# ahuang73/HemoCell

Hardware: AMD Instinct MI355X
Metric: MLUPS + cell-vertex updates/s, 256^3 pipeflow 10% Hct (higher is better)
Workload: dtype f64

## Files before the change

### hemocell_amd/csrc/common.h

```cpp
#pragma once
#include <hip/hip_runtime.h>
#include <stdint.h>
#include <string>
#include <vector>
#include "../../include/hemocell_amd.h"

namespace hc {

void set_error(const std::string &msg);
int hip_fail(hipError_t e, const char *what, const char *file, int line);
hipStream_t stream();
hipStream_t comm_stream();
int fork();
void route(int side);
int join();
bool forked();

#define HC_HIP(call)                                                         \
  do {                                                                       \
    hipError_t e__ = (call);                                                 \
    if (e__ != hipSuccess) return hc::hip_fail(e__, #call, __FILE__, __LINE__); \
  } while (0)

#define HC_REQUIRE(cond, msg)                 \
  do {                                        \
    if (!(cond)) {                            \
      hc::set_error(std::string(msg));        \
      return HC_ERR_ARG;                      \
    }                                         \
  } while (0)

enum ProfKernel { PK_COLLIDE = 0, PK_SPREAD, PK_INTERP, PK_ADVANCE, PK_MECH, PK_COLLIDE_BESIDE, PK_LEES_EDWARDS, PK_COUNT };
struct ProfScope {
  int k; bool on;
  hipEvent_t a, b;
  explicit ProfScope(int kernel);
  ~ProfScope();
};

#define HC_CX {0, -1, 0, 0, -1, -1, -1, -1, 0, 0, 1, 0, 0, 1, 1, 1, 1, 0, 0}
#define HC_CY {0, 0, -1, 0, -1, 1, 0, 0, -1, -1, 0, 1, 0, 1, -1, 0, 0, 1, 1}
#define HC_CZ {0, 0, 0, -1, 0, 0, -1, 1, -1, 1, 0, 0, 1, 0, 0, 1, -1, 1, -1}

constexpr int HALO = 2;

constexpr int STAT_BLOCKS = 512;
struct StatAcc { double mn, mx, sum; long n; };
__device__ __forceinline__ void stat_add(StatAcc &a, double v) { a.mn = v < a.mn ? v : a.mn; a.mx = v > a.mx ? v : a.mx; a.sum += v; a.n++; }
__device__ __forceinline__ void stat_block_store(StatAcc a, double *partial ) {
  __shared__ double s_red[4][4];
#pragma unroll
  for (int off = 32; off > 0; off >>= 1) {
    const double mn = __shfl_xor(a.mn, off), mx = __shfl_xor(a.mx, off), sm = __shfl_xor(a.sum, off);
    const long n = __shfl_xor(a.n, off);
    a.mn = mn < a.mn ? mn : a.mn; a.mx = mx > a.mx ? mx : a.mx; a.sum += sm; a.n += n;
  }
  const int w = threadIdx.x >> 6;
  if ((threadIdx.x & 63) == 0) { s_red[w][0] = a.mn; s_red[w][1] = a.mx; s_red[w][2] = a.sum; s_red[w][3] = (double)a.n; }
  __syncthreads();
  if (threadIdx.x == 0) {
    double mn = s_red[0][0], mx = s_red[0][1], sm = s_red[0][2], n = s_red[0][3];
    for (int k = 1; k < (int)(blockDim.x >> 6); k++) { mn = s_red[k][0] < mn ? s_red[k][0] : mn; mx = s_red[k][1] > mx ? s_red[k][1] : mx; sm += s_red[k][2]; n += s_red[k][3]; }
    double *o = partial + 4 * blockIdx.x;
    o[0] = mn; o[1] = mx; o[2] = sm; o[3] = n;
  }
}
int stat_finish(const double *d_partial, double out[3], long *n, double *h_pinned = nullptr);

}

namespace hc {
struct BodyRegions { int n; int box[HC_MAX_FORCE_REGIONS][6]; double f[HC_MAX_FORCE_REGIONS][3]; };
#ifdef __HIPCC__
__device__ __forceinline__ void region_force(const BodyRegions &r, int xg, int y, int z, double &bx, double &by, double &bz) {
  for (int k = 0; k < r.n; k++) {
    const int *b = r.box[k];
    if (xg >= b[0] && xg <= b[1] && y >= b[2] && y <= b[3] && z >= b[4] && z <= b[5]) { bx = r.f[k][0]; by = r.f[k][1]; bz = r.f[k][2]; }
  }
}

__device__ __forceinline__ void zou_he_x(double f[HC_Q], int code, const double *__restrict__ val) {
  const int kind = code & 3;
  const long slot = code >> 2;
  const double s0 = f[0] + f[2] + f[3] + f[8] + f[9] + f[11] + f[12] + f[17] + f[18];
  const double sm = f[1] + f[4] + f[5] + f[6] + f[7];
  const double sp = f[10] + f[13] + f[14] + f[15] + f[16];
  const bool neg = (kind & 1) == 0;
  const double s_out = neg ? sm : sp;
  const double known = s0 + 2.0 * s_out + 1.0;
  double rho, ux, uy, uz;
  if (kind < 2) {
    ux = val[4 * slot]; uy = val[4 * slot + 1]; uz = val[4 * slot + 2];
    rho = neg ? known / (1.0 - ux) : known / (1.0 + ux);
  } else {
    rho = val[4 * slot + 3];
    ux = neg ? 1.0 - known / rho : known / rho - 1.0;
    uy = 0.0; uz = 0.0;
  }
  const double ny = 0.5 * ((f[11] + f[17] + f[18]) - (f[2] + f[8] + f[9])) - rho * uy / 3.0;
  const double nz = 0.5 * ((f[12] + f[9] + f[17]) - (f[3] + f[8] + f[18])) - rho * uz / 3.0;
  if (neg) {
    f[10] = f[1] + rho * ux / 3.0;
    f[13] = f[4] + rho * (ux + uy) / 6.0 - ny;
    f[14] = f[5] + rho * (ux - uy) / 6.0 + ny;
    f[15] = f[6] + rho * (ux + uz) / 6.0 - nz;
    f[16] = f[7] + rho * (ux - uz) / 6.0 + nz;
  } else {
    f[1] = f[10] - rho * ux / 3.0;
    f[4] = f[13] - rho * (ux + uy) / 6.0 + ny;
    f[5] = f[14] - rho * (ux - uy) / 6.0 - ny;
    f[6] = f[15] - rho * (ux + uz) / 6.0 + nz;
    f[7] = f[16] - rho * (ux - uz) / 6.0 - nz;
  }
}
#endif
}

struct hc_lattice {
  int nx, ny, nz;
  int periodic[3];
  int x0, nx_global, n_slabs;
  double omega;
  size_t plane;
  size_t xs;
  size_t npad;
  size_t qstride;
  double *f[2];
  int cur;
  double *force[3];
  int fcur;
  int ibm;
  uint8_t *fdirty[3];
  uint8_t fepoch[3];
  uint8_t *wallbrick; int nbx, nby, nbz;
  uint8_t *mask;
  std::vector<uint8_t> hmask;
  double body[3];
  hc::BodyRegions regions;
  double wall_u[4][3];
  int *row_z0, *row_cum, *blk_row;
  int nblk, max_active;
  double *scratch;
  size_t scratch_doubles;
  double *halo_u[2] = {nullptr, nullptr};
  bool halo_u_valid = false;
  bool le_on = false;
  double le_D = 0.0, le_d = 0.0, le_v_top = 0.0, le_v_bottom = 0.0;
  double *le_buf = nullptr;
  int *ob_code = nullptr;
  std::vector<int> ob_hcode;
  double *ob_val = nullptr;
  int ob_n = 0, ob_cap = 0;
  int *ob_list = nullptr; int ob_list_cap = 0;
  double *ob_out = nullptr; int ob_out_cap = 0;
};

namespace hc {
int lees_edwards_step(hc_lattice *L);
}

namespace hcs {
int iterate_slab(hc_lattice *L, hc_cells *C, long *iter, int n, int particle_timescale, int force_limit);
int collide_stream_slab(hc_lattice *L, int nsteps);
void lattice_destroyed(hc_lattice *L);
void halos_stale(hc_lattice *L);
void set_overlap(int on);
}
```

### hemocell_amd/csrc/lattice.hip

```cpp
#include "common.h"
#include "comm.h"
#include <algorithm>
#include <type_traits>

using namespace hc;

namespace {

struct LatArgs {
  const double *fin;
  double *fout;
  const double *Fin;
  double *Fzero;
  const uint8_t *mask;
  int nx, ny, nz;
  int plane;
  long xs;
  long npad;
  long qs;
  int x_begin;
  int x_split, x_jump;
  int wrap_x, per_y, per_z;
  double omega;
  double bx, by, bz;
  const int *row_z0, *row_cum, *blk_row;
  int nblk;
  int ibm;
  const uint8_t *dirty_in, *dirty_zero; uint8_t epoch_in, epoch_zero;
  double wall_u[4][3];
  int x0, nx_global;
  BodyRegions reg;
};

struct OpenArgs : LatArgs {
  const int *ob_code;
  const double *ob_val;
};
template <bool OPEN> using Args = std::conditional_t<OPEN, OpenArgs, LatArgs>;

__device__ __forceinline__ void body_at(const LatArgs &a, int x, int y, int z, double &bx, double &by, double &bz) {
  bx = a.bx; by = a.by; bz = a.bz;
  if (a.reg.n) region_force(a.reg, a.x0 + x, y, z, bx, by, bz);
}

struct Nbr {
  long xm, xp;
  int ym, yp, zm, zp;
  bool ym_ok, yp_ok, zm_ok, zp_ok;
};

__device__ __forceinline__ Nbr neighbours(const LatArgs &a, int x, int y, int z) {
  Nbr n;
  n.xm = -a.xs; n.xp = a.xs;
  if (a.wrap_x) {
    if (x == 0) n.xm = (long)(a.nx - 1) * a.xs;
    if (x == a.nx - 1) n.xp = -(long)(a.nx - 1) * a.xs;
  }
  n.ym = -a.nz; n.yp = a.nz; n.ym_ok = n.yp_ok = true;
  if (y == 0) { if (a.per_y) n.ym = (a.ny - 1) * a.nz; else n.ym_ok = false; }
  if (y == a.ny - 1) { if (a.per_y) n.yp = -(a.ny - 1) * a.nz; else n.yp_ok = false; }
  n.zm = -1; n.zp = 1; n.zm_ok = n.zp_ok = true;
  if (z == 0) { if (a.per_z) n.zm = a.nz - 1; else n.zm_ok = false; }
  if (z == a.nz - 1) { if (a.per_z) n.zp = -(a.nz - 1); else n.zp_ok = false; }
  return n;
}

template <int CX, int CY, int CZ>
__device__ __forceinline__ long src_off(const Nbr &n, bool &ok) {
  long off = 0; ok = true;
  if (CX == 1) off += n.xm; else if (CX == -1) off += n.xp;
  if (CY == 1) { off += n.ym; ok = ok && n.ym_ok; } else if (CY == -1) { off += n.yp; ok = ok && n.yp_ok; }
  if (CZ == 1) { off += n.zm; ok = ok && n.zm_ok; } else if (CZ == -1) { off += n.zp; ok = ok && n.zp_ok; }
  return off;
}
template <int CX, int CY, int CZ>
__device__ __forceinline__ long dst_off(const Nbr &n, bool &ok) {
  long off = 0; ok = true;
  if (CX == 1) off += n.xp; else if (CX == -1) off += n.xm;
  if (CY == 1) { off += n.yp; ok = ok && n.yp_ok; } else if (CY == -1) { off += n.ym; ok = ok && n.ym_ok; }
  if (CZ == 1) { off += n.zp; ok = ok && n.zp_ok; } else if (CZ == -1) { off += n.zm; ok = ok && n.zm_ok; }
  return off;
}

#define FOR_Q(M)                                                                                     \
  M(0, 0, 0, 0) M(1, -1, 0, 0) M(2, 0, -1, 0) M(3, 0, 0, -1) M(4, -1, -1, 0) M(5, -1, 1, 0)          \
  M(6, -1, 0, -1) M(7, -1, 0, 1) M(8, 0, -1, -1) M(9, 0, -1, 1) M(10, 1, 0, 0) M(11, 0, 1, 0)        \
  M(12, 0, 0, 1) M(13, 1, 1, 0) M(14, 1, -1, 0) M(15, 1, 0, 1) M(16, 1, 0, -1) M(17, 0, 1, 1)        \
  M(18, 0, 1, -1)

__device__ __forceinline__ constexpr double tq(int q) { return q == 0 ? 1. / 3. : ((q >= 1 && q <= 3) || (q >= 10 && q <= 12)) ? 1. / 18. : 1. / 36.; }

__device__ __forceinline__ void pull(const double *__restrict__ fin, long npad, long node, const Nbr &n, double f[HC_Q]) {
#define M(Q, CX, CY, CZ)                                   \
  {                                                        \
    bool ok; long off = src_off<CX, CY, CZ>(n, ok);        \
    f[Q] = ok ? fin[(long)Q * npad + node + off] : 0.0;    \
  }
  FOR_Q(M)
#undef M
}

template <bool OPEN>
__device__ __forceinline__ void complete_open(const Args<OPEN> &a, long node, double f[HC_Q]) {
  if constexpr (OPEN) {
    if (a.mask[node] == 0) {
      const int code = a.ob_code[node];
      if (code >= 0) zou_he_x(f, code, a.ob_val);
    }
  }
}

__device__ __forceinline__ void moments(const double f[HC_Q], double &rhoBar, double &jx, double &jy, double &jz) {
  double r = 0.0, x = 0.0, y = 0.0, z = 0.0;
#define M(Q, CX, CY, CZ)              \
  r += f[Q];                          \
  if (CX == 1) x += f[Q]; else if (CX == -1) x += -f[Q]; \
  if (CY == 1) y += f[Q]; else if (CY == -1) y += -f[Q]; \
  if (CZ == 1) z += f[Q]; else if (CZ == -1) z += -f[Q];
  FOR_Q(M)
#undef M
  rhoBar = r; jx = x; jy = y; jz = z;
}

template <int CX, int CY, int CZ>
__device__ __forceinline__ double cdot(double a0, double a1, double a2) {
  double s = 0.0; bool first = true;
  if (CX != 0) { s = (CX == 1 ? a0 : -a0); first = false; }
  if (CY != 0) { double t = (CY == 1 ? a1 : -a1); s = first ? t : s + t; first = false; }
  if (CZ != 0) { double t = (CZ == 1 ? a2 : -a2); s = first ? t : s + t; first = false; }
  return s;
}

__device__ __forceinline__ void collide_guo(double f[HC_Q], double Fx, double Fy, double Fz, double omega) {
  double rhoBar, j0, j1, j2;
  moments(f, rhoBar, j0, j1, j2);
  const double invRho = 1.0 / (1.0 + rhoBar);
  const double rho = 1.0 + rhoBar;
  const double u0 = j0 * invRho + Fx / 2.0, u1 = j1 * invRho + Fy / 2.0, u2 = j2 * invRho + Fz / 2.0;
  j0 = rho * u0; j1 = rho * u1; j2 = rho * u2;
  const double jSqr = j0 * j0 + j1 * j1 + j2 * j2;
  const double one_m_omega = 1.0 - omega;
  const double guo = 1.0 - omega / 2.0;
#define M(Q, CX, CY, CZ)                                                                     \
  {                                                                                          \
    const double c_j = cdot<CX, CY, CZ>(j0, j1, j2);                                         \
    const double feq = tq(Q) * (rhoBar + 3.0 * c_j + invRho * (4.5 * c_j * c_j - 1.5 * jSqr)); \
    f[Q] *= one_m_omega;                                                                     \
    f[Q] += omega * feq;                                                                     \
  }
  FOR_Q(M)
#undef M
#define M(Q, CX, CY, CZ)                                                                     \
  {                                                                                          \
    double c_u = cdot<CX, CY, CZ>(u0, u1, u2);                                               \
    c_u *= 9.0;                                                                              \
    double ft = (((double)CX - u0) * 3.0 + c_u * (double)CX) * Fx;                           \
    ft += (((double)CY - u1) * 3.0 + c_u * (double)CY) * Fy;                                 \
    ft += (((double)CZ - u2) * 3.0 + c_u * (double)CZ) * Fz;                                 \
    ft *= tq(Q);                                                                             \
    ft *= guo;                                                                               \
    f[Q] += ft;                                                                              \
  }
  FOR_Q(M)
#undef M
}

template <bool REGIONS, bool OPEN = false>
__global__ __launch_bounds__(256) void collide_stream_kernel(Args<OPEN> a) {
  const int x = a.x_begin + (int)blockIdx.y + ((int)blockIdx.y >= a.x_split ? a.x_jump : 0);
  const int xp = x + HALO;
  const int t = blockIdx.x * 256 + threadIdx.x;
  const int *cum = a.row_cum + (long)xp * (a.ny + 1);
  if (t >= cum[a.ny]) return;
  int lo = a.blk_row[(long)xp * (a.nblk + 1) + blockIdx.x], hi = a.blk_row[(long)xp * (a.nblk + 1) + blockIdx.x + 1];
  while (lo < hi) { const int mid = (lo + hi + 1) >> 1; if (cum[mid] <= t) lo = mid; else hi = mid - 1; }
  const int y = lo, z = a.row_z0[(long)xp * a.ny + y] + (t - cum[y]);
  const int p = y * a.nz + z;
  const long node = (long)(x + HALO) * a.xs + p;
  const uint8_t m = a.mask[node];
  if (m == 2) return;
  const Nbr n = neighbours(a, x, y, z);
  const bool fdirty = a.ibm && m == 0 && a.dirty_in[node >> 4] == a.epoch_in;
  double F0 = 0.0, F1 = 0.0, F2 = 0.0;
  if (fdirty) { F0 = a.Fin[3 * node]; F1 = a.Fin[3 * node + 1]; F2 = a.Fin[3 * node + 2]; }
  double f[HC_Q];
  pull(a.fin, a.qs, node, n, f);
  const bool wall = m != 0;
  if (wall) {
#pragma unroll
    for (int i = 1; i <= 9; i++) { double t = f[i]; f[i] = f[i + 9]; f[i + 9] = t; }
    if (m >= 3) {
      const double w0 = a.wall_u[m - 3][0], w1 = a.wall_u[m - 3][1], w2 = a.wall_u[m - 3][2];
#define M(Q, CX, CY, CZ)                                                                  \
      if (Q != 0) {                                                                       \
        constexpr int O = Q <= 9 ? Q + 9 : Q - 9;                                         \
        const double c_u = (double)CX * w0 + (double)CY * w1 + (double)CZ * w2;           \
        f[O] = f[O] - 6.0 * tq(Q) * c_u;                                                  \
      }
      FOR_Q(M)
#undef M
    }
  } else {
    double bx = a.bx, by = a.by, bz = a.bz;
    if (REGIONS) region_force(a.reg, a.x0 + x, y, z, bx, by, bz);
    double Fx = bx, Fy = by, Fz = bz;
    if (fdirty) {
      Fx = bx + F0; Fy = by + F1; Fz = bz + F2;
    }
    if constexpr (OPEN) {
      const int code = a.ob_code[node];
      if (code >= 0) zou_he_x(f, code, a.ob_val);
    }
    collide_guo(f, Fx, Fy, Fz, a.omega);
  }
#pragma unroll
  for (int q = 0; q < HC_Q; q++) __builtin_nontemporal_store(f[q], &a.fout[(long)q * a.qs + node]);
  if (a.ibm && a.dirty_zero[node >> 4] == a.epoch_zero) { a.Fzero[3 * node] = 0.0; a.Fzero[3 * node + 1] = 0.0; a.Fzero[3 * node + 2] = 0.0; }
}

__global__ void init_eq_kernel(LatArgs a, double rhoBar, double j0, double j1, double j2) {
  const int p = blockIdx.x * 256 + threadIdx.x;
  if (p >= a.plane) return;
  const int x = a.x_begin + blockIdx.y;
  const int y = p / a.nz, z = p - y * a.nz;
  const long node = (long)(x + HALO) * a.xs + p;
  const Nbr n = neighbours(a, x, y, z);
  const double invRho = 1.0 / (1.0 + rhoBar);
  const double jSqr = j0 * j0 + j1 * j1 + j2 * j2;
#define M(Q, CX, CY, CZ)                                                                        \
  {                                                                                             \
    bool ok; long off = dst_off<CX, CY, CZ>(n, ok);                                             \
    double v = 0.0;                                                                             \
    if (ok && a.mask[node + off] == 0) {                                                        \
      const double c_j = cdot<CX, CY, CZ>(j0, j1, j2);                                          \
      v = tq(Q) * (rhoBar + 3.0 * c_j + invRho * (4.5 * c_j * c_j - 1.5 * jSqr));               \
    }                                                                                           \
    a.fout[(long)Q * a.qs + node] = v;                                                          \
  }
  FOR_Q(M)
#undef M
}

__global__ void download_kernel(LatArgs a, double *aos) {
  const int p = blockIdx.x * 256 + threadIdx.x;
  if (p >= a.plane) return;
  const int x = a.x_begin + blockIdx.y;
  const int y = p / a.nz, z = p - y * a.nz;
  const long node = (long)(x + HALO) * a.xs + p;
  const Nbr n = neighbours(a, x, y, z);
  double f[HC_Q];
  pull(a.fin, a.qs, node, n, f);
  const long o = ((long)x * a.plane + p) * HC_Q;
#pragma unroll
  for (int q = 0; q < HC_Q; q++) aos[o + q] = f[q];
}

__global__ void upload_kernel(LatArgs a, const double *aos, int lo_ok, int hi_ok) {
  const int p = blockIdx.x * 256 + threadIdx.x;
  if (p >= a.plane) return;
  const int x = a.x_begin + blockIdx.y;
  const int y = p / a.nz, z = p - y * a.nz;
  const long node = (long)(x + HALO) * a.xs + p;
  const long bulk = (long)x * a.plane + p;
  Nbr nl = neighbours(a, x, y, z);
  nl.xm = nl.xm / a.xs * a.plane; nl.xp = nl.xp / a.xs * a.plane;
#define M(Q, CX, CY, CZ)                                                                  \
  {                                                                                       \
    bool ok; long off = dst_off<CX, CY, CZ>(nl, ok);                                      \
     \
    if (!a.wrap_x && ((CX == 1 && x == a.nx - 1 && !hi_ok) || (CX == -1 && x == 0 && !lo_ok))) ok = false; \
    a.fout[(long)Q * a.qs + node] = ok ? aos[(bulk + off) * HC_Q + Q] : 0.0;            \
  }
  FOR_Q(M)
#undef M
}

template <bool OPEN = false>
__global__ void rho_u_kernel(Args<OPEN> a, double *rho, double *u) {
  const int p = blockIdx.x * 256 + threadIdx.x;
  if (p >= a.plane) return;
  const int x = a.x_begin + blockIdx.y;
  const int y = p / a.nz, z = p - y * a.nz;
  const long node = (long)(x + HALO) * a.xs + p;
  const Nbr n = neighbours(a, x, y, z);
  double f[HC_Q];
  pull(a.fin, a.qs, node, n, f);
  complete_open<OPEN>(a, node, f);
  double rhoBar, j0, j1, j2;
  moments(f, rhoBar, j0, j1, j2);
  const double invRho = 1.0 / (1.0 + rhoBar);
  const long o = (long)x * a.plane + p;
  rho[o] = 1.0 + rhoBar;
  double bx, by, bz;
  body_at(a, x, y, z, bx, by, bz);
  u[3 * o] = j0 * invRho + (bx + a.Fin[3 * node]) / 2.0;
  u[3 * o + 1] = j1 * invRho + (by + a.Fin[3 * node + 1]) / 2.0;
  u[3 * o + 2] = j2 * invRho + (bz + a.Fin[3 * node + 2]) / 2.0;
}

template <bool OPEN = false>
__global__ void pi_neq_kernel(Args<OPEN> a, double *pi) {
  const int p = blockIdx.x * 256 + threadIdx.x;
  if (p >= a.plane) return;
  const int x = a.x_begin + blockIdx.y;
  const int y = p / a.nz, z = p - y * a.nz;
  const long node = (long)(x + HALO) * a.xs + p;
  const Nbr n = neighbours(a, x, y, z);
  double f[HC_Q];
  pull(a.fin, a.qs, node, n, f);
  complete_open<OPEN>(a, node, f);
  double rhoBar, j0, j1, j2;
  moments(f, rhoBar, j0, j1, j2);
  const double invRho = 1.0 / (1.0 + rhoBar);
  double xx = 0, xy = 0, xz = 0, yy = 0, yz = 0, zz = 0;
#define M(Q, CX, CY, CZ)                       \
  if (CX * CX) xx += f[Q];                     \
  if (CX * CY == 1) xy += f[Q]; else if (CX * CY == -1) xy += -f[Q]; \
  if (CX * CZ == 1) xz += f[Q]; else if (CX * CZ == -1) xz += -f[Q]; \
  if (CY * CY) yy += f[Q];                     \
  if (CY * CZ == 1) yz += f[Q]; else if (CY * CZ == -1) yz += -f[Q]; \
  if (CZ * CZ) zz += f[Q];
  FOR_Q(M)
#undef M
  const double cs2 = 1.0 / 3.0;
  const long o = 6 * ((long)x * a.plane + p);
  pi[o] = xx - invRho * j0 * j0 - cs2 * rhoBar;
  pi[o + 1] = xy - invRho * j0 * j1;
  pi[o + 2] = xz - invRho * j0 * j2;
  pi[o + 3] = yy - invRho * j1 * j1 - cs2 * rhoBar;
  pi[o + 4] = yz - invRho * j1 * j2;
  pi[o + 5] = zz - invRho * j2 * j2 - cs2 * rhoBar;
}

template <bool OPEN = false>
__global__ void plane_velocity_kernel(Args<OPEN> a, int x, const int *yz, int n, double *out) {
  const int k = blockIdx.x * 256 + threadIdx.x;
  if (k >= n) return;
  const int p = yz[k];
  const int y = p / a.nz, z = p - y * a.nz;
  const long node = (long)(x + HALO) * a.xs + p;
  double u0 = 0.0, u1 = 0.0, u2 = 0.0;
  if (a.mask[node] == 0) {
    const Nbr nb = neighbours(a, x, y, z);
    double f[HC_Q];
    pull(a.fin, a.qs, node, nb, f);
    complete_open<OPEN>(a, node, f);
    double rhoBar, j0, j1, j2;
    moments(f, rhoBar, j0, j1, j2);
    const double invRho = 1.0 / (1.0 + rhoBar);
    double bx, by, bz;
    body_at(a, x, y, z, bx, by, bz);
    u0 = j0 * invRho + bx / 2.0; u1 = j1 * invRho + by / 2.0; u2 = j2 * invRho + bz / 2.0;
  }
  out[3L * k] = u0; out[3L * k + 1] = u1; out[3L * k + 2] = u2;
}

__global__ void ob_set_kernel(double *val, int first, int n, const double *src, int c0, int nc) {
  const int k = blockIdx.x * 256 + threadIdx.x;
  if (k >= n * nc) return;
  const int i = k / nc, c = k - i * nc;
  val[4L * (first + i) + c0 + c] = src[k];
}

__global__ void force_aos_kernel(LatArgs a, double *F) {
  const int p = blockIdx.x * 256 + threadIdx.x;
  if (p >= a.plane) return;
  const int x = a.x_begin + blockIdx.y;
  const long node = (long)(x + HALO) * a.xs + p;
  const long o = (long)x * a.plane + p;
  for (int d = 0; d < 3; d++) F[3 * o + d] = a.Fin[3 * node + d];
// ... 3 lines not shown
__global__ __launch_bounds__(256) void fluid_stats_kernel(Args<OPEN> a, int what, double *partial) {
  StatAcc acc{1e300, -1e300, 0.0, 0};
  const long nbulk = (long)a.nx * a.plane;
  for (long k = (long)blockIdx.x * 256 + threadIdx.x; k < nbulk; k += (long)STAT_BLOCKS * 256) {
    const int x = (int)(k / a.plane), p = (int)(k - (long)x * a.plane);
    const long node = (long)(x + HALO) * a.xs + p;
    if (what == 2) {
      double r = 0.0;
#pragma unroll
      for (int q = 0; q < HC_Q; q++) r += a.fin[(long)q * a.qs + node];
      stat_add(acc, r);
      continue;
    }
    if (a.mask[node] != 0) continue;
    const int y = p / a.nz, z = p - y * a.nz;
    double bx, by, bz;
    body_at(a, x, y, z, bx, by, bz);
    double Fx = bx, Fy = by, Fz = bz;
    if (a.ibm) { Fx = bx + a.Fin[3 * node]; Fy = by + a.Fin[3 * node + 1]; Fz = bz + a.Fin[3 * node + 2]; }
    double v0 = Fx, v1 = Fy, v2 = Fz;
    if (what == 0) {
      const Nbr n = neighbours(a, x, y, z);
      double f[HC_Q];
      pull(a.fin, a.qs, node, n, f);
      complete_open<OPEN>(a, node, f);
      double rhoBar, j0, j1, j2;
      moments(f, rhoBar, j0, j1, j2);
      const double invRho = 1.0 / (1.0 + rhoBar);
      v0 = j0 * invRho + Fx / 2.0; v1 = j1 * invRho + Fy / 2.0; v2 = j2 * invRho + Fz / 2.0;
    }
    stat_add(acc, sqrt(v0 * v0 + v1 * v1 + v2 * v2));
  }
  stat_block_store(acc, partial);
}


__device__ __forceinline__ void collide_external(double f[HC_Q], double rhoBar, double j0, double j1, double j2, double omega) {
  const double invRho = 1.0 / (1.0 + rhoBar);
  const double jSqr = j0 * j0 + j1 * j1 + j2 * j2;
  const double one_m_omega = 1.0 - omega;
#define M(Q, CX, CY, CZ)                                                                     \
  {                                                                                          \
    const double c_j = cdot<CX, CY, CZ>(j0, j1, j2);                                         \
    const double feq = tq(Q) * (rhoBar + 3.0 * c_j + invRho * (4.5 * c_j * c_j - 1.5 * jSqr)); \
    f[Q] *= one_m_omega;                                                                     \
    f[Q] += omega * feq;                                                                     \
  }
  FOR_Q(M)
#undef M
}

__device__ __forceinline__ long modp(long a, long b) { return (a % b + b) % b; }

__global__ __launch_bounds__(256) void le_gather_kernel(LatArgs a, double *buf, double D, double v_top, double v_bottom) {
  const long nxy = (long)a.nx * a.ny;
  const long t = (long)blockIdx.x * 256 + threadIdx.x;
  if (t >= 2 * nxy) return;
  const int top = t < nxy ? 1 : 0;
  const long r = top ? t : t - nxy;
  const int x = (int)(r / a.ny), y = (int)(r - (long)x * a.ny);
  const int z = top ? a.nz - 1 : 0;
  const long row = (long)y * a.nz + z;
  const long node = (long)(x + HALO) * a.xs + row;
  double f[HC_Q];
  pull(a.fin, a.qs, node, neighbours(a, x, y, z), f);
  double rhoBar = 0.0;
#pragma unroll
  for (int q = 0; q < HC_Q; q++) rhoBar += f[q];
  collide_external(f, rhoBar, top ? v_top : v_bottom, 0.0, 0.0, a.omega);
  const double g = fmod(D, 1.0);
  const long s1 = top ? modp((long)ceil(D + (double)x), a.nx) : modp((long)floor(-D + (double)x), a.nx);
  const long s2 = top ? modp((long)floor(D + (double)x), a.nx) : modp((long)ceil(-D + (double)x), a.nx);
  double f1[HC_Q], f2[HC_Q];
  pull(a.fin, a.qs, (s1 + HALO) * a.xs + row, neighbours(a, (int)s1, y, z), f1);
  pull(a.fin, a.qs, (s2 + HALO) * a.xs + row, neighbours(a, (int)s2, y, z), f2);
  if (top) {
    f[3] = g * f1[3] + (1 - g) * f2[3];
    f[6] = g * f1[16] + (1 - g) * f2[16];
    f[8] = g * f1[8] + (1 - g) * f2[8];
    f[16] = g * f1[6] + (1 - g) * f2[6];
    f[18] = g * f1[18] + (1 - g) * f2[18];
  } else {
    f[7] = g * f1[15] + (1 - g) * f2[15];
    f[9] = g * f1[9] + (1 - g) * f2[9];
    f[12] = g * f1[12] + (1 - g) * f2[12];
    f[15] = g * f1[7] + (1 - g) * f2[7];
    f[17] = g * f1[17] + (1 - g) * f2[17];
  }
  double *o = buf + (long)(1 - top) * HC_Q * nxy + r;
#pragma unroll
  for (int q = 0; q < HC_Q; q++) o[(long)q * nxy] = f[q];
}

__global__ __launch_bounds__(256) void le_scatter_kernel(LatArgs a, const double *buf) {
  const long nxy = (long)a.nx * a.ny;
  const long t = (long)blockIdx.x * 256 + threadIdx.x;
  if (t >= 2 * nxy) return;
  const int top = t < nxy ? 1 : 0;
  const long r = top ? t : t - nxy;
  const int x = (int)(r / a.ny), y = (int)(r - (long)x * a.ny);
  const int z = top ? a.nz - 1 : 0;
  const long node = (long)(x + HALO) * a.xs + (long)y * a.nz + z;
  const Nbr n = neighbours(a, x, y, z);
  const double *in = buf + (long)(1 - top) * HC_Q * nxy + r;
#define M(Q, CX, CY, CZ)                                                       \
  {                                                                            \
    bool ok; const long off = src_off<CX, CY, CZ>(n, ok);                      \
    if (ok) a.fout[(long)Q * a.qs + node + off] = in[(long)Q * nxy];           \
  }
  FOR_Q(M)
#undef M
}

struct HaloArgs {
  double *f;
  double *buf;
  double *buf2; int n_first;
  long npad; long xs; int plane;
  int n;
  int pop[HC_Q + 5];
  int xp[HC_Q + 5];
  int to_buf;
};
__global__ void halo_copy_kernel(HaloArgs h) {
  const int p = blockIdx.x * 256 + threadIdx.x;
  if (p >= h.plane) return;
  const int e = blockIdx.y;
  const long li = (long)h.pop[e] * h.npad + (long)h.xp[e] * h.xs + p;
  double *b = e < h.n_first ? h.buf + (long)e * h.plane + p : h.buf2 + (long)(e - h.n_first) * h.plane + p;
  if (h.to_buf) *b = h.f[li]; else h.f[li] = *b;
}

__global__ void zero_force_halo_kernel(double *F, long xs, int plane, int nx) {
  const int e = blockIdx.x * 256 + threadIdx.x;
  if (e >= 3 * plane) return;
  const int w = blockIdx.y;
  const int xp = w < HALO ? w : nx + w;
  F[3 * (long)xp * xs + e] = 0.0;
}

LatArgs make_args(const hc_lattice *L) {
  LatArgs a;
  a.fin = L->f[L->cur]; a.fout = L->f[1 - L->cur];
  const int fprev = (L->fcur + 2) % 3;
  a.Fin = L->force[L->fcur]; a.Fzero = L->force[fprev];
  a.x_split = 0x7fffffff; a.x_jump = 0;
  a.mask = L->mask;
  a.nx = L->nx; a.ny = L->ny; a.nz = L->nz; a.plane = (int)L->plane; a.xs = (long)L->xs; a.npad = (long)L->npad; a.qs = (long)L->qstride;
  a.x_begin = 0;
  a.wrap_x = (L->n_slabs == 1 && L->periodic[0]) ? 1 : 0;
  a.per_y = L->periodic[1]; a.per_z = L->periodic[2];
  a.omega = L->omega; a.bx = L->body[0]; a.by = L->body[1]; a.bz = L->body[2];
  a.x0 = L->x0; a.nx_global = L->nx_global; a.reg = L->regions;
  a.row_z0 = L->row_z0; a.row_cum = L->row_cum; a.blk_row = L->blk_row; a.nblk = L->nblk;
  a.ibm = L->ibm;
  a.dirty_in = L->fdirty[L->fcur]; a.dirty_zero = L->fdirty[fprev]; a.epoch_in = L->fepoch[L->fcur]; a.epoch_zero = L->fepoch[fprev];
  for (int c = 0; c < 4; c++) for (int d = 0; d < 3; d++) a.wall_u[c][d] = L->wall_u[c][d];
  return a;
}

OpenArgs open_args(const hc_lattice *L, const LatArgs &a) {
  OpenArgs o;
  static_cast<LatArgs &>(o) = a;
  o.ob_code = L->ob_code; o.ob_val = L->ob_val;
  return o;
}

dim3 plane_grid(const hc_lattice *L, int nplanes) { return dim3((unsigned)((L->plane + 255) / 256), (unsigned)nplanes, 1); }

int ensure_scratch(hc_lattice *L, size_t doubles) {
  if (L->scratch_doubles >= doubles) return HC_OK;
  if (L->scratch) HC_HIP(hipFree(L->scratch));
  L->scratch = nullptr; L->scratch_doubles = 0;
  HC_HIP(hipMalloc((void **)&L->scratch, doubles * sizeof(double)));
  L->scratch_doubles = doubles;
  return HC_OK;
}

int rebuild_active_map(hc_lattice *L) {
  const int NX = L->nx + 2 * HALO, ny = L->ny, nz = L->nz;
  std::vector<int> z0((size_t)NX * ny), cum((size_t)NX * (ny + 1));
  int max_active = 0;
  for (int x = 0; x < NX; x++) {
    int c = 0;
    for (int y = 0; y < ny; y++) {
      const uint8_t *row = L->hmask.data() + (size_t)x * L->xs + (size_t)y * nz;
      int a = 0, b = nz;
      while (a < nz && row[a] == 2) a++;
      while (b > a && row[b - 1] == 2) b--;
      z0[(size_t)x * ny + y] = a;
      cum[(size_t)x * (ny + 1) + y] = c;
      c += b - a;
    }
    cum[(size_t)x * (ny + 1) + ny] = c;
    max_active = std::max(max_active, c);
  }
  if (max_active == 0) max_active = 1;
  const int nblk = (max_active + 255) / 256;
  std::vector<int> blk((size_t)NX * (nblk + 1));
  for (int x = 0; x < NX; x++) {
    const int *cx = cum.data() + (size_t)x * (ny + 1);
    int y = 0;
    for (int b = 0; b <= nblk; b++) {
      const long t = (long)b * 256;
      while (y + 1 < ny && cx[y + 1] <= t) y++;
      blk[(size_t)x * (nblk + 1) + b] = y;
    }
  }
  for (int **p : {&L->row_z0, &L->row_cum, &L->blk_row}) if (*p) { HC_HIP(hipFree(*p)); *p = nullptr; }
  HC_HIP(hipMalloc((void **)&L->row_z0, z0.size() * sizeof(int)));
  HC_HIP(hipMalloc((void **)&L->row_cum, cum.size() * sizeof(int)));
  HC_HIP(hipMalloc((void **)&L->blk_row, blk.size() * sizeof(int)));
  HC_HIP(hipMemcpy(L->row_z0, z0.data(), z0.size() * sizeof(int), hipMemcpyHostToDevice));
  HC_HIP(hipMemcpy(L->row_cum, cum.data(), cum.size() * sizeof(int), hipMemcpyHostToDevice));
  HC_HIP(hipMemcpy(L->blk_row, blk.data(), blk.size() * sizeof(int), hipMemcpyHostToDevice));
  L->nblk = nblk; L->max_active = max_active;
  return HC_OK;
}

int rebuild_wall_bricks(hc_lattice *L) {
  const int NX = L->nx + 2 * HALO, ny = L->ny, nz = L->nz;
  std::vector<uint8_t> flag((size_t)L->nbx * L->nby * L->nbz, 0);
  for (int bx = 0; bx < L->nbx; bx++)
    for (int by = 0; by < L->nby; by++)
      for (int bz = 0; bz < L->nbz; bz++) {
        bool near = false;
        if (!L->periodic[1] && (by == 0 || by == L->nby - 1)) near = true;
        if (!L->periodic[2] && (bz == 0 || bz == L->nbz - 1)) near = true;
        if (bx * 8 < HALO + 1 || bx * 8 + 7 >= L->nx + HALO - 1) near = true;
        for (int x = bx * 8; x < std::min(NX, bx * 8 + 8) && !near; x++)
          for (int y = by * 8; y < std::min(ny, by * 8 + 8) && !near; y++) {
            const uint8_t *row = L->hmask.data() + (size_t)x * L->xs + (size_t)y * nz;
            for (int z = bz * 8; z < std::min(nz, bz * 8 + 8); z++) if (row[z] != 0) { near = true; break; }
          }
        flag[((size_t)bx * L->nby + by) * L->nbz + bz] = near ? 1 : 0;
      }
  if (!L->wallbrick) HC_HIP(hipMalloc((void **)&L->wallbrick, flag.size()));
  HC_HIP(hipMemcpy(L->wallbrick, flag.data(), flag.size(), hipMemcpyHostToDevice));
  return HC_OK;
}

int launch_collide(hc_lattice *L, int x_begin, int nplanes, int x2 = 0, int n2 = 0) {
  if (nplanes + n2 <= 0) return HC_OK;
  LatArgs a = make_args(L);
  a.x_begin = x_begin;
  if (n2 > 0) { a.x_split = nplanes; a.x_jump = x2 - (x_begin + nplanes); }
  const unsigned ny = (unsigned)(nplanes + n2);
  const dim3 grid((unsigned)((L->max_active + 255) / 256), ny, 1);
  if (L->ob_n > 0) {
    const OpenArgs o = open_args(L, a);
    if (L->regions.n) hipLaunchKernelGGL((collide_stream_kernel<true, true>), grid, dim3(256), 0, hc::stream(), o);
    else hipLaunchKernelGGL((collide_stream_kernel<false, true>), grid, dim3(256), 0, hc::stream(), o);
  } else if (L->regions.n) hipLaunchKernelGGL(collide_stream_kernel<true>, grid, dim3(256), 0, hc::stream(), a);
  else hipLaunchKernelGGL(collide_stream_kernel<false>, grid, dim3(256), 0, hc::stream(), a);
  HC_HIP(hipGetLastError());
  return HC_OK;
}

int launch_lees_edwards(hc_lattice *L) {
  hc::ProfScope prof(hc::PK_LEES_EDWARDS);
  LatArgs a = make_args(L);
  a.fout = L->f[L->cur];
  const long nthreads = 2L * L->nx * L->ny;
  const dim3 grid((unsigned)((nthreads + 255) / 256));
  hipLaunchKernelGGL(le_gather_kernel, grid, dim3(256), 0, hc::stream(), a, L->le_buf, L->le_D, L->le_v_top, L->le_v_bottom);
  HC_HIP(hipGetLastError());
  hipLaunchKernelGGL(le_scatter_kernel, grid, dim3(256), 0, hc::stream(), a, (const double *)L->le_buf);
  HC_HIP(hipGetLastError());
  return HC_OK;
}

}

int hc::lees_edwards_step(hc_lattice *L) { return L->le_on ? launch_lees_edwards(L) : HC_OK; }

static bool le_layers_fluid(const hc_lattice *L, const uint8_t *mask, size_t xs) {
  const int zs[4] = {0, 1, L->nz - 2, L->nz - 1};
  for (int x = HALO; x < L->nx + HALO; x++)
    for (int y = 0; y < L->ny; y++)
      for (int k = 0; k < 4; k++)
        if (mask[(size_t)x * xs + (size_t)y * L->nz + zs[k]] != 0) return false;
  return true;
}

static int g_force_plane_padding = 0;

extern "C" {

int hc_debug_force_plane_padding(int on) { g_force_plane_padding = on > 0 ? 1 : (on < 0 ? -1 : 0); return HC_OK; }

int hcl_create(hc_lattice **out, int nx, int ny, int nz, const int periodic[3], double omega,
               int x0, int nx_global, int n_slabs) {
  HC_REQUIRE(out && periodic, "hcl_create: null pointer");
  HC_REQUIRE(nx >= 2 && ny >= 2 && nz >= 2, "hcl_create: every dimension must be >= 2");
  HC_REQUIRE(n_slabs >= 1 && nx_global >= nx && x0 >= 0 && x0 + nx <= nx_global, "hcl_create: inconsistent slab decomposition");
  HC_REQUIRE((long)ny * nz < (1L << 30) && (long)(nx + 2 * HALO) * (((long)ny + 8) * nz + 32) < (1L << 31), "hcl_create: slab too large for 32-bit plane indexing");
  HC_REQUIRE(omega > 0.0 && omega < 2.0, "hcl_create: omega must be in (0,2)");
  if (hc::stream() == nullptr) { hc::set_error("hcl_create: hc_init() has not been called"); return HC_ERR_STATE; }
  hc_lattice *L = new hc_lattice();
  L->nx = nx; L->ny = ny; L->nz = nz;
  for (int d = 0; d < 3; d++) L->periodic[d] = periodic[d] ? 1 : 0;
  L->x0 = x0; L->nx_global = nx_global; L->n_slabs = n_slabs;
  L->omega = omega;
  L->plane = (size_t)ny * nz;
  L->xs = (L->plane + 15) / 16 * 16;
  if (g_force_plane_padding > 0 || (g_force_plane_padding == 0 && ((L->plane * sizeof(double)) % (1u << 20)) == 0)) L->xs += (size_t)(8 * nz + 15) / 16 * 16;
  if (g_force_plane_padding < 0) L->xs = L->plane;
  L->npad = (size_t)(nx + 2 * HALO) * L->xs;
  L->qstride = L->npad + 16 * 129;
  L->cur = 0; L->fcur = 0; L->ibm = 0;
  L->body[0] = L->body[1] = L->body[2] = 0.0;
  L->regions.n = 0;
  for (int c = 0; c < 4; c++) for (int d = 0; d < 3; d++) L->wall_u[c][d] = 0.0;
  L->scratch = nullptr; L->scratch_doubles = 0;
  L->f[0] = L->f[1] = nullptr; L->mask = nullptr;
  for (int k = 0; k < 3; k++) { L->force[k] = nullptr; L->fdirty[k] = nullptr; }
  for (int k = 0; k < 2; k++) {
    HC_HIP(hipMalloc((void **)&L->f[k], L->qstride * HC_Q * sizeof(double)));
    HC_HIP(hipMemsetAsync(L->f[k], 0, L->qstride * HC_Q * sizeof(double), hc::stream()));
  }
  for (int k = 0; k < 3; k++) {
    HC_HIP(hipMalloc((void **)&L->force[k], L->npad * 3 * sizeof(double)));
    HC_HIP(hipMemsetAsync(L->force[k], 0, L->npad * 3 * sizeof(double), hc::stream()));
  }
  HC_HIP(hipMalloc((void **)&L->mask, L->npad));
  HC_HIP(hipMemsetAsync(L->mask, 0, L->npad, hc::stream()));
  for (int k = 0; k < 3; k++) {
    HC_HIP(hipMalloc((void **)&L->fdirty[k], L->npad / 16 + 1));
    HC_HIP(hipMemsetAsync(L->fdirty[k], 0, L->npad / 16 + 1, hc::stream()));
    L->fepoch[k] = 1;
  }
  L->hmask.assign(L->npad, 0);
  L->row_z0 = L->row_cum = L->blk_row = nullptr;
  L->wallbrick = nullptr; L->nbx = (nx + 2 * HALO + 7) / 8; L->nby = (ny + 7) / 8; L->nbz = (nz + 7) / 8;
  { int rc = rebuild_active_map(L); if (rc != HC_OK) return rc; }
  { int rc = rebuild_wall_bricks(L); if (rc != HC_OK) return rc; }
  HC_HIP(hipStreamSynchronize(hc::stream()));
  *out = L;
  return HC_OK;
}

int hcl_destroy(hc_lattice *L) {
  if (!L) return HC_OK;
  hcs::lattice_destroyed(L);
  hipStreamSynchronize(hc::stream());
  for (int k = 0; k < 2; k++) if (L->f[k]) hipFree(L->f[k]);
  for (int k = 0; k < 3; k++) { if (L->force[k]) hipFree(L->force[k]); if (L->fdirty[k]) hipFree(L->fdirty[k]); }
  if (L->mask) hipFree(L->mask);
  if (L->scratch) hipFree(L->scratch);
  if (L->row_z0) hipFree(L->row_z0);
  if (L->row_cum) hipFree(L->row_cum);
  if (L->blk_row) hipFree(L->blk_row);
  if (L->wallbrick) hipFree(L->wallbrick);
  if (L->le_buf) hipFree(L->le_buf);
  if (L->ob_code) hipFree(L->ob_code);
  if (L->ob_val) hipFree(L->ob_val);
  if (L->ob_list) hipFree(L->ob_list);
  if (L->ob_out) hipFree(L->ob_out);
  delete L;
  return HC_OK;
}

int hcl_dims(const hc_lattice *L, int dims[3]) {
  HC_REQUIRE(L && dims, "hcl_dims: null pointer");
  dims[0] = L->nx; dims[1] = L->ny; dims[2] = L->nz;
  return HC_OK;
}

int hcl_node_counts(const hc_lattice *L, long counts[3]) {
  HC_REQUIRE(L && counts, "hcl_node_counts: null pointer");
  long fluid = 0, active = 0;
  for (int x = 0; x < L->nx; x++)
    for (size_t p = 0; p < L->plane; p++) {
      const uint8_t m = L->hmask[(size_t)(x + HALO) * L->xs + p];
      fluid += m == 0; active += m != 2;
    }
  counts[0] = (long)L->nx * (long)L->plane; counts[1] = fluid; counts[2] = active;
  return HC_OK;
}

int hcl_set_mask(hc_lattice *L, const uint8_t *mask_with_halo) {
  HC_REQUIRE(L && mask_with_halo, "hcl_set_mask: null pointer");
  if (L->le_on && !le_layers_fluid(L, mask_with_halo, L->plane)) {
    hc::set_error("hcl_set_mask: the lattice has a Lees-Edwards boundary; the layers z = 0, 1, nz-2 and nz-1 must hold fluid nodes only");
    return HC_ERR_STATE;
  }
  L->hmask.assign(L->npad, 2);
  for (int x = 0; x < L->nx + 2 * HALO; x++)
    for (size_t p = 0; p < L->plane; p++) {
      const uint8_t m = mask_with_halo[(size_t)x * L->plane + p];
      L->hmask[(size_t)x * L->xs + p] = (m >= 3 && m <= 6) ? m : (m ? 1 : 0);
    }
  {
    static const int cx[HC_Q] = HC_CX, cy[HC_Q] = HC_CY, cz[HC_Q] = HC_CZ;
    const int NX = L->nx + 2 * HALO, ny = L->ny, nz = L->nz;
    std::vector<uint8_t> cls(L->hmask);
    for (int x = 0; x < NX; x++)
      for (int y = 0; y < ny; y++)
        for (int z = 0; z < nz; z++) {
          const size_t k = (size_t)x * L->xs + (size_t)y * nz + z;
          if (!L->hmask[k]) continue;
          bool fluid_near = false;
          for (int q = 1; q < HC_Q && !fluid_near; q++) {
            int xx = x + cx[q], yy = y + cy[q], zz = z + cz[q];
            if (xx < 0 || xx >= NX) { fluid_near = true; break; }
            if (yy < 0 || yy >= ny) { if (L->periodic[1]) yy = (yy + ny) % ny; else continue; }
            if (zz < 0 || zz >= nz) { if (L->periodic[2]) zz = (zz + nz) % nz; else continue; }
            if (!L->hmask[(size_t)xx * L->xs + (size_t)yy * nz + zz]) fluid_near = true;
          }
          if (!fluid_near) cls[k] = 2;
        }
    const size_t n = cls.size();
    for (size_t g = 0; g < n; g += 16) {
      const size_t e = std::min(n, g + 16);
      bool live = false;
      for (size_t k = g; k < e; k++) if (cls[k] != 2) { live = true; break; }
      if (live) for (size_t k = g; k < e; k++) if (cls[k] == 2) cls[k] = 1;
    }
    L->hmask.swap(cls);
  }
  { int rc = rebuild_active_map(L); if (rc != HC_OK) return rc; }
  { int rc = rebuild_wall_bricks(L); if (rc != HC_OK) return rc; }
  HC_HIP(hipMemcpyAsync(L->mask, L->hmask.data(), L->npad, hipMemcpyHostToDevice, hc::stream()));
  HC_HIP(hipStreamSynchronize(hc::stream()));
  return HC_OK;
}

int hcl_init_equilibrium(hc_lattice *L, double rho, const double u[3]) {
  HC_REQUIRE(L && u, "hcl_init_equilibrium: null pointer");
  LatArgs a = make_args(L);
  a.fout = L->f[L->cur];
  HC_HIP(hipMemsetAsync(L->f[0], 0, L->qstride * HC_Q * sizeof(double), hc::stream()));
  HC_HIP(hipMemsetAsync(L->f[1], 0, L->qstride * HC_Q * sizeof(double), hc::stream()));
  hipLaunchKernelGGL(init_eq_kernel, plane_grid(L, L->nx), dim3(256), 0, hc::stream(), a, rho - 1.0, rho * u[0], rho * u[1], rho * u[2]);
  HC_HIP(hipGetLastError());
  HC_HIP(hipStreamSynchronize(hc::stream()));
  return HC_OK;
}

int hcl_set_wall_velocity(hc_lattice *L, int wall_class, const double u[3]) {
  HC_REQUIRE(L && u && wall_class >= 3 && wall_class <= 6, "hcl_set_wall_velocity: class must be 3..6");
  for (int d = 0; d < 3; d++) L->wall_u[wall_class - 3][d] = u[d];
  return HC_OK;
}

int hcl_set_body_force(hc_lattice *L, const double F[3]) {
  HC_REQUIRE(L && F, "hcl_set_body_force: null pointer");
  for (int d = 0; d < 3; d++) L->body[d] = F[d];
  return HC_OK;
}

int hcl_set_body_force_regions(hc_lattice *L, int n, const int *boxes, const double *forces) {
  HC_REQUIRE(L && n >= 0 && (n == 0 || (boxes && forces)), "hcl_set_body_force_regions: bad arguments");
  HC_REQUIRE(n <= HC_MAX_FORCE_REGIONS, "hcl_set_body_force_regions: more than HC_MAX_FORCE_REGIONS boxes");
  for (int k = 0; k < n; k++) {
    const int *b = boxes + 6 * k;
    HC_REQUIRE(b[0] <= b[1] && b[2] <= b[3] && b[4] <= b[5], "hcl_set_body_force_regions: empty box");
    for (int i = 0; i < 6; i++) L->regions.box[k][i] = b[i];
    for (int d = 0; d < 3; d++) L->regions.f[k][d] = forces[3 * k + d];
  }
  L->regions.n = n;
  return HC_OK;
}

int hcl_collide_stream_part(hc_lattice *L, int part) {
  HC_REQUIRE(L, "hcl_collide_stream_part: null lattice");
  HC_REQUIRE(part >= 0 && part <= 6, "hcl_collide_stream_part: part must be 0..6");
  HC_REQUIRE(part < 3 || L->nx >= 4, "hcl_collide_stream_part: parts 3, 4 and 6 need a slab of at least 4 planes");
  hc::ProfScope prof(hc::forked() ? hc::PK_COLLIDE_BESIDE : hc::PK_COLLIDE);
  int rc = HC_OK;
  if (part == 0) rc = launch_collide(L, 0, L->nx);
  else if (part == 1) rc = launch_collide(L, 1, L->nx - 2);
  else if (part == 2 || part == 5) rc = launch_collide(L, 0, 1, L->nx - 1, 1);
  else if (part == 3) rc = launch_collide(L, 2, L->nx - 4);
  else rc = launch_collide(L, 0, 2, L->nx - 2, 2);
  if (rc == HC_OK && (part == 0 || part == 2 || part == 4)) rc = hcl_zero_force_halos(L);
  return rc;
}

int hcl_zero_force_halos(hc_lattice *L) {
  HC_REQUIRE(L, "hcl_zero_force_halos: null lattice");
  if (L->n_slabs <= 1 || !L->ibm) return HC_OK;
  hipLaunchKernelGGL(zero_force_halo_kernel, dim3((unsigned)((3 * L->plane + 255) / 256), (unsigned)(2 * HALO), 1), dim3(256), 0, hc::stream(),
                     L->force[(L->fcur + 2) % 3], (long)L->xs, (int)L->plane, L->nx);
  HC_HIP(hipGetLastError());
  return HC_OK;
}

int hcl_step_end(hc_lattice *L) {
  HC_REQUIRE(L, "hcl_step_end: null lattice");
  L->cur ^= 1; L->fcur = (L->fcur + 1) % 3;
  L->halo_u_valid = false;
  L->fepoch[L->fcur] = (uint8_t)(L->fepoch[L->fcur] % 255 + 1);
  return HC_OK;
}

int hcl_collide_stream(hc_lattice *L, int nsteps) {
  HC_REQUIRE(L, "hcl_collide_stream: null lattice");
  if (L->n_slabs > 1) return hcs::collide_stream_slab(L, nsteps);
  for (int s = 0; s < nsteps; s++) {
    int rc = hcl_collide_stream_part(L, 0);
    if (rc != HC_OK) return rc;
    hcl_step_end(L);
    if ((rc = hc::lees_edwards_step(L)) != HC_OK) return rc;
  }
// ... 353 lines not shown
```

Measured before the change: 16740.

## Replace per-thread row binary search with packed block descriptors and wave readlane scan

Replaces the row_z0/row_cum/blk_row tables with a per-block int4 descriptor (first row, row count, live threads) and a packed int2 per-row table (cumulative start, z offset). Each thread now finds its row with a wave-wide readlane scan instead of a dependent binary search through global memory. The kernel also issues the mask, dirty-flag, open-boundary code and distribution loads earlier, makes the pull loads unconditional with a clamped offset, and pins occupancy with amdgpu_waves_per_eu. The intent is to shorten the dependent load chain at kernel start and raise memory-level parallelism. In exchange, every thread does a serial scan over the block's rows, and fully-masked (m==2) nodes now perform the loads and collision work before exiting.

```diff
diff --git a/hemocell_amd/csrc/common.h b/hemocell_amd/csrc/common.h
--- a/hemocell_amd/csrc/common.h
+++ b/hemocell_amd/csrc/common.h
@@ -138,7 +138,7 @@
   double body[3];
   hc::BodyRegions regions;
   double wall_u[4][3];
-  int *row_z0, *row_cum, *blk_row;
+  int *blk_desc, *row_pack;
   int nblk, max_active;
   double *scratch;
   size_t scratch_doubles;
diff --git a/hemocell_amd/csrc/lattice.hip b/hemocell_amd/csrc/lattice.hip
--- a/hemocell_amd/csrc/lattice.hip
+++ b/hemocell_amd/csrc/lattice.hip
@@ -10,25 +10,27 @@
 struct LatArgs {
   const double *fin;
   double *fout;
+  const uint8_t *mask;
+  const int4 *blk_desc;
+  const int2 *row_pack;
+  const uint8_t *dirty_in, *dirty_zero;
   const double *Fin;
   double *Fzero;
-  const uint8_t *mask;
+  long xs;
+  long qs;
   int nx, ny, nz;
-  int plane;
-  long xs;
-  long npad;
-  long qs;
+  int nblk;
   int x_begin;
   int x_split, x_jump;
   int wrap_x, per_y, per_z;
+  int ibm;
+  uint8_t epoch_in, epoch_zero;
   double omega;
   double bx, by, bz;
-  const int *row_z0, *row_cum, *blk_row;
-  int nblk;
-  int ibm;
-  const uint8_t *dirty_in, *dirty_zero; uint8_t epoch_in, epoch_zero;
+  int plane;
+  long npad;
+  int x0, nx_global;
   double wall_u[4][3];
-  int x0, nx_global;
   BodyRegions reg;
 };
 
@@ -51,11 +53,8 @@
 
 __device__ __forceinline__ Nbr neighbours(const LatArgs &a, int x, int y, int z) {
   Nbr n;
-  n.xm = -a.xs; n.xp = a.xs;
-  if (a.wrap_x) {
-    if (x == 0) n.xm = (long)(a.nx - 1) * a.xs;
-    if (x == a.nx - 1) n.xp = -(long)(a.nx - 1) * a.xs;
-  }
+  n.xm = (a.wrap_x && x == 0) ? (long)(a.nx - 1) * a.xs : -a.xs;
+  n.xp = (a.wrap_x && x == a.nx - 1) ? -(long)(a.nx - 1) * a.xs : a.xs;
   n.ym = -a.nz; n.yp = a.nz; n.ym_ok = n.yp_ok = true;
   if (y == 0) { if (a.per_y) n.ym = (a.ny - 1) * a.nz; else n.ym_ok = false; }
   if (y == a.ny - 1) { if (a.per_y) n.yp = -(a.ny - 1) * a.nz; else n.yp_ok = false; }
@@ -91,10 +90,11 @@
 __device__ __forceinline__ constexpr double tq(int q) { return q == 0 ? 1. / 3. : ((q >= 1 && q <= 3) || (q >= 10 && q <= 12)) ? 1. / 18. : 1. / 36.; }
 
 __device__ __forceinline__ void pull(const double *__restrict__ fin, long npad, long node, const Nbr &n, double f[HC_Q]) {
-#define M(Q, CX, CY, CZ)                                   \
-  {                                                        \
-    bool ok; long off = src_off<CX, CY, CZ>(n, ok);        \
-    f[Q] = ok ? fin[(long)Q * npad + node + off] : 0.0;    \
+#define M(Q, CX, CY, CZ)                                             \
+  {                                                                  \
+    bool ok; long off = src_off<CX, CY, CZ>(n, ok);                  \
+    const double v = fin[(long)Q * npad + node + (ok ? off : 0)];    \
+    f[Q] = ok ? v : 0.0;                                             \
   }
   FOR_Q(M)
 #undef M
@@ -165,26 +165,42 @@
 #undef M
 }
 
+template <class T> __device__ __forceinline__ void fetch_now(const T &v) { asm volatile("" ::"s"(v)); }
+template <class T, class... U> __device__ __forceinline__ void fetch_now(const T &v, const U &...w) { fetch_now(v); fetch_now(w...); }
+
 template <bool REGIONS, bool OPEN = false>
-__global__ __launch_bounds__(256) void collide_stream_kernel(Args<OPEN> a) {
+__global__ __launch_bounds__(256) __attribute__((amdgpu_waves_per_eu(4, 4))) void collide_stream_kernel(Args<OPEN> a) {
   const int x = a.x_begin + (int)blockIdx.y + ((int)blockIdx.y >= a.x_split ? a.x_jump : 0);
   const int xp = x + HALO;
-  const int t = blockIdx.x * 256 + threadIdx.x;
-  const int *cum = a.row_cum + (long)xp * (a.ny + 1);
-  if (t >= cum[a.ny]) return;
-  int lo = a.blk_row[(long)xp * (a.nblk + 1) + blockIdx.x], hi = a.blk_row[(long)xp * (a.nblk + 1) + blockIdx.x + 1];
-  while (lo < hi) { const int mid = (lo + hi + 1) >> 1; if (cum[mid] <= t) lo = mid; else hi = mid - 1; }
-  const int y = lo, z = a.row_z0[(long)xp * a.ny + y] + (t - cum[y]);
+  const int4 d = a.blk_desc[(long)xp * a.nblk + blockIdx.x];
+  fetch_now(a.nx, a.ny, a.nz, a.ibm, a.wrap_x, a.per_y, a.per_z, (int)a.epoch_in, (int)a.epoch_zero, a.xs, a.qs, a.fin, a.fout, a.Fin, a.Fzero,
+            a.mask, a.dirty_in, a.dirty_zero, a.row_pack, a.omega, a.bx, a.by, a.bz);
+  if (d.z == 0) return;
+  const int t = blockIdx.x * 256 + threadIdx.x, lane = threadIdx.x & 63;
+  const int2 *rows = a.row_pack + (long)xp * a.ny + d.x;
+  int y = d.x, zoff = 0;
+  for (int base = 0; base < d.y; base += 64) {
+    const int2 r = rows[min(base + lane, d.y - 1)];
+    const int cnt = min(64, d.y - base);
+    for (int k = 0; k < cnt; k++) {
+      const int c = __builtin_amdgcn_readlane(r.x, k), o = __builtin_amdgcn_readlane(r.y, k);
+      if (c <= t) { y = d.x + base + k; zoff = o; }
+    }
+  }
+  if ((int)threadIdx.x >= d.z) return;
+  const int z = t + zoff;
   const int p = y * a.nz + z;
-  const long node = (long)(x + HALO) * a.xs + p;
+  const long node = (long)xp * a.xs + p;
   const uint8_t m = a.mask[node];
-  if (m == 2) return;
+  const uint8_t d_in = a.dirty_in[node >> 4], d_zero = a.dirty_zero[node >> 4];
+  int code = -1;
+  if constexpr (OPEN) code = a.ob_code[node];
   const Nbr n = neighbours(a, x, y, z);
-  const bool fdirty = a.ibm && m == 0 && a.dirty_in[node >> 4] == a.epoch_in;
+  double f[HC_Q];
+  pull(a.fin, a.qs, node, n, f);
+  const bool fdirty = a.ibm && m == 0 && d_in == a.epoch_in;
   double F0 = 0.0, F1 = 0.0, F2 = 0.0;
   if (fdirty) { F0 = a.Fin[3 * node]; F1 = a.Fin[3 * node + 1]; F2 = a.Fin[3 * node + 2]; }
-  double f[HC_Q];
-  pull(a.fin, a.qs, node, n, f);
   const bool wall = m != 0;
   if (wall) {
 #pragma unroll
@@ -208,14 +224,14 @@
       Fx = bx + F0; Fy = by + F1; Fz = bz + F2;
     }
     if constexpr (OPEN) {
-      const int code = a.ob_code[node];
       if (code >= 0) zou_he_x(f, code, a.ob_val);
     }
     collide_guo(f, Fx, Fy, Fz, a.omega);
   }
+  if (m == 2) return;
 #pragma unroll
   for (int q = 0; q < HC_Q; q++) __builtin_nontemporal_store(f[q], &a.fout[(long)q * a.qs + node]);
-  if (a.ibm && a.dirty_zero[node >> 4] == a.epoch_zero) { a.Fzero[3 * node] = 0.0; a.Fzero[3 * node + 1] = 0.0; a.Fzero[3 * node + 2] = 0.0; }
+  if (a.ibm && d_zero == a.epoch_zero) { a.Fzero[3 * node] = 0.0; a.Fzero[3 * node + 1] = 0.0; a.Fzero[3 * node + 2] = 0.0; }
 }
 
 __global__ void init_eq_kernel(LatArgs a, double rhoBar, double j0, double j1, double j2) {
@@ -525,7 +541,7 @@
   a.per_y = L->periodic[1]; a.per_z = L->periodic[2];
   a.omega = L->omega; a.bx = L->body[0]; a.by = L->body[1]; a.bz = L->body[2];
   a.x0 = L->x0; a.nx_global = L->nx_global; a.reg = L->regions;
-  a.row_z0 = L->row_z0; a.row_cum = L->row_cum; a.blk_row = L->blk_row; a.nblk = L->nblk;
+  a.blk_desc = (const int4 *)L->blk_desc; a.row_pack = (const int2 *)L->row_pack; a.nblk = L->nblk;
   a.ibm = L->ibm;
   a.dirty_in = L->fdirty[L->fcur]; a.dirty_zero = L->fdirty[fprev]; a.epoch_in = L->fepoch[L->fcur]; a.epoch_zero = L->fepoch[fprev];
   for (int c = 0; c < 4; c++) for (int d = 0; d < 3; d++) a.wall_u[c][d] = L->wall_u[c][d];
@@ -570,23 +586,30 @@
   }
   if (max_active == 0) max_active = 1;
   const int nblk = (max_active + 255) / 256;
-  std::vector<int> blk((size_t)NX * (nblk + 1));
+  std::vector<int> desc((size_t)NX * nblk * 4, 0), pack((size_t)NX * ny * 2);
   for (int x = 0; x < NX; x++) {
     const int *cx = cum.data() + (size_t)x * (ny + 1);
+    for (int y = 0; y < ny; y++) {
+      pack[((size_t)x * ny + y) * 2] = cx[y];
+      pack[((size_t)x * ny + y) * 2 + 1] = z0[(size_t)x * ny + y] - cx[y];
+    }
     int y = 0;
-    for (int b = 0; b <= nblk; b++) {
+    for (int b = 0; b < nblk; b++) {
       const long t = (long)b * 256;
+      const int live = (int)std::min<long>(256, std::max<long>(0, cx[ny] - t));
+      if (live == 0) continue;
       while (y + 1 < ny && cx[y + 1] <= t) y++;
-      blk[(size_t)x * (nblk + 1) + b] = y;
-    }
-  }
-  for (int **p : {&L->row_z0, &L->row_cum, &L->blk_row}) if (*p) { HC_HIP(hipFree(*p)); *p = nullptr; }
-  HC_HIP(hipMalloc((void **)&L->row_z0, z0.size() * sizeof(int)));
-  HC_HIP(hipMalloc((void **)&L->row_cum, cum.size() * sizeof(int)));
-  HC_HIP(hipMalloc((void **)&L->blk_row, blk.size() * sizeof(int)));
-  HC_HIP(hipMemcpy(L->row_z0, z0.data(), z0.size() * sizeof(int), hipMemcpyHostToDevice));
-  HC_HIP(hipMemcpy(L->row_cum, cum.data(), cum.size() * sizeof(int), hipMemcpyHostToDevice));
-  HC_HIP(hipMemcpy(L->blk_row, blk.data(), blk.size() * sizeof(int), hipMemcpyHostToDevice));
+      int last = y;
+      while (last + 1 < ny && cx[last + 1] <= t + live - 1) last++;
+      int *d = desc.data() + ((size_t)x * nblk + b) * 4;
+      d[0] = y; d[1] = last - y + 1; d[2] = live;
+    }
+  }
+  for (int **p : {&L->blk_desc, &L->row_pack}) if (*p) { HC_HIP(hipFree(*p)); *p = nullptr; }
+  HC_HIP(hipMalloc((void **)&L->blk_desc, desc.size() * sizeof(int)));
+  HC_HIP(hipMalloc((void **)&L->row_pack, pack.size() * sizeof(int)));
+  HC_HIP(hipMemcpy(L->blk_desc, desc.data(), desc.size() * sizeof(int), hipMemcpyHostToDevice));
+  HC_HIP(hipMemcpy(L->row_pack, pack.data(), pack.size() * sizeof(int), hipMemcpyHostToDevice));
   L->nblk = nblk; L->max_active = max_active;
   return HC_OK;
 }
@@ -704,7 +727,7 @@
     L->fepoch[k] = 1;
   }
   L->hmask.assign(L->npad, 0);
-  L->row_z0 = L->row_cum = L->blk_row = nullptr;
+  L->blk_desc = L->row_pack = nullptr;
   L->wallbrick = nullptr; L->nbx = (nx + 2 * HALO + 7) / 8; L->nby = (ny + 7) / 8; L->nbz = (nz + 7) / 8;
   { int rc = rebuild_active_map(L); if (rc != HC_OK) return rc; }
   { int rc = rebuild_wall_bricks(L); if (rc != HC_OK) return rc; }
@@ -721,9 +744,8 @@
   for (int k = 0; k < 3; k++) { if (L->force[k]) hipFree(L->force[k]); if (L->fdirty[k]) hipFree(L->fdirty[k]); }
   if (L->mask) hipFree(L->mask);
   if (L->scratch) hipFree(L->scratch);
-  if (L->row_z0) hipFree(L->row_z0);
-  if (L->row_cum) hipFree(L->row_cum);
-  if (L->blk_row) hipFree(L->blk_row);
+  if (L->blk_desc) hipFree(L->blk_desc);
+  if (L->row_pack) hipFree(L->row_pack);
   if (L->wallbrick) hipFree(L->wallbrick);
   if (L->le_buf) hipFree(L->le_buf);
   if (L->ob_code) hipFree(L->ob_code);
```

Result: slower. 15740 (-6.0%).
